# Kainmueller-Lab/PatchPerPix

Hardware: AMD Instinct MI355X
Metric: Mvoxels/sec assembled (vote_instances) (higher is better)
Workload: dtype f16 in, f32 accumulate

## Files before the change

include/ppp_mi355x.h:

```cpp
#ifndef PPP_MI355X_H
#define PPP_MI355X_H

#include <stddef.h>
#include <stdint.h>

#ifdef __cplusplus
extern "C" {
#endif

#define PPP_ABI_VERSION 5

enum ppp_error {
    PPP_OK = 0,
    PPP_ERR_INVALID_ARG = -1,
    PPP_ERR_NO_DEVICE = -2,
    PPP_ERR_HIP = -3,
    PPP_ERR_UNSUPPORTED = -4,
    PPP_ERR_WORKSPACE = -5
};

enum ppp_dtype { PPP_F32 = 0, PPP_F16 = 1, PPP_BF16 = 2 };

enum ppp_bg_rule { PPP_BG_INV_TH = 0, PPP_BG_HALF_TH = 1, PPP_BG_LESS_THAN_TH = 2 };
enum ppp_value_rule { PPP_VAL_COUNT = 0, PPP_VAL_PROB_PRODUCT = 1, PPP_VAL_NORM_PROB_PRODUCT = 2 };
// ... 44 lines not shown
int ppp_consensus_writes_voxel_major(const ppp_params *p);
int ppp_consensus_rows(const void *d_pred, int pred_dtype, const uint8_t *d_overlap, float *d_cons,
                       const ppp_params *p, void *stream);

int ppp_consensus_part(const void *d_pred, int pred_dtype, const uint8_t *d_overlap, float *d_cons,
                       const ppp_params *p, const ppp_box *part, void *stream);

int64_t ppp_consensus_sparse_workspace_bytes(const ppp_params *p, const ppp_box *part);
int ppp_consensus_sparse(const void *d_pred, int pred_dtype, const uint8_t *d_overlap, float *d_cons,
                         float *d_count, const ppp_params *p, const ppp_box *part, int open_rows, void *d_work,
                         int mode, void *stream);
void ppp_consensus_last_items(int64_t *total, int64_t *active, int *took_lists);

int ppp_rank_patches(const void *d_pred, int pred_dtype, const float *d_cons,
                     const uint8_t *d_overlap, float *d_score, const ppp_box *score_box,
                     const ppp_params *p, void *stream);

int64_t ppp_rank_workspace_bytes(const ppp_box *score_box, const ppp_params *p);
int ppp_rank_patches_vm(const void *d_pred, int pred_dtype, const float *d_cons_vm,
                        const uint8_t *d_overlap, float *d_score, const ppp_box *score_box,
                        void *d_work, const ppp_params *p, void *stream);
int ppp_rank_wg_plan(const ppp_box *score_box, const ppp_params *p, int resident_per_cu, int cus_per_xcd,
                     int32_t plan[8]);

int ppp_patch_graph(const void *d_pred, int pred_dtype, const float *d_cons,
                    const uint32_t *d_pairs, const uint32_t *d_order, uint64_t n_pairs,
                    float *d_aff, const ppp_params *p, void *stream);

int32_t ppp_patch_graph_by_patch_chunk(const ppp_params *p);
int32_t ppp_patch_graph_by_patch_chunk_small(const ppp_params *p);
int ppp_patch_graph_by_patch_chunked(const void *d_pred, int pred_dtype, const float *d_cons_vm,
                                     const uint32_t *d_pairs, const uint32_t *d_order,
                                     const int64_t *d_group_start, const int64_t *d_chunk_offsets,
                                     int32_t n_groups, int64_t n_blocks, int32_t chunk, float *d_aff,
                                     const ppp_params *p, void *stream);
int64_t ppp_patch_graph_lcg_words(int32_t dz, int32_t dy, int32_t dx, const ppp_params *p);
int ppp_patch_graph_lcg(const void *d_pred, int pred_dtype, const uint32_t *d_pairs,
                        const uint32_t *d_order, const int64_t *d_lcg_pos, int64_t n_lcg,
                        const int64_t *d_drop_off, uint64_t *d_drops, const ppp_params *p, void *stream);
int ppp_patch_graph_by_patch_lcg(const void *d_pred, int pred_dtype, const float *d_cons_vm,
                                 const uint32_t *d_pairs, const uint32_t *d_order,
                                 const int64_t *d_group_start, const int64_t *d_chunk_offsets,
                                 int32_t n_groups, int64_t n_blocks, int32_t chunk, float *d_aff,
                                 const int64_t *d_drop_off, const uint64_t *d_drops,
                                 const ppp_params *p, void *stream);
int ppp_patch_fg_bits(const void *d_pred, int pred_dtype, const int64_t *d_centres, int64_t n,
// ... 295 lines not shown
```

patchperpix_amd/backend.py:

```python
import ctypes
import os

import numpy as np

from . import build as _build

F32, F16, BF16 = 0, 1, 2
BG_INV_TH, BG_HALF_TH, BG_LESS_THAN_TH = 0, 1, 2
VAL_COUNT, VAL_PROB_PRODUCT, VAL_NORM_PROB_PRODUCT = 0, 1, 2
CONS_COMPACT, CONS_REFERENCE, CONS_VOXEL_MAJOR = 0, 1, 2
ABI_VERSION = 5
NONE_KEY = 0xFFFFFFFF
NONE_KEY64 = 1 << 62
PAIR_KEY_FAR = 0x7FFFFFFFFFFFFFFF


class Box(ctypes.Structure):
    _fields_ = [(n, ctypes.c_int32) for n in ("z0", "y0", "x0", "z1", "y1", "x1")]

    def shape(self):
        return (self.z1 - self.z0, self.y1 - self.y0, self.x1 - self.x0)


class Params(ctypes.Structure):
# ... 60 lines not shown
    "ppp_consensus": (ctypes.c_int, [ctypes.c_void_p, ctypes.c_int, ctypes.c_void_p,
                                     ctypes.c_void_p, ctypes.c_void_p,
                                     ctypes.POINTER(Params), ctypes.c_void_p]),
    "ppp_consensus_rows": (ctypes.c_int, [ctypes.c_void_p, ctypes.c_int, ctypes.c_void_p,
                                          ctypes.c_void_p, ctypes.POINTER(Params), ctypes.c_void_p]),
    "ppp_consensus_part": (ctypes.c_int, [ctypes.c_void_p, ctypes.c_int, ctypes.c_void_p,
                                          ctypes.c_void_p, ctypes.POINTER(Params), ctypes.POINTER(Box),
                                          ctypes.c_void_p]),
    "ppp_consensus_sparse_workspace_bytes": (ctypes.c_int64, [ctypes.POINTER(Params), ctypes.POINTER(Box)]),
    "ppp_consensus_sparse": (ctypes.c_int, [ctypes.c_void_p, ctypes.c_int, ctypes.c_void_p, ctypes.c_void_p,
                                            ctypes.c_void_p, ctypes.POINTER(Params), ctypes.POINTER(Box),
                                            ctypes.c_int, ctypes.c_void_p, ctypes.c_int, ctypes.c_void_p]),
    "ppp_consensus_last_items": (None, [ctypes.POINTER(ctypes.c_int64), ctypes.POINTER(ctypes.c_int64),
                                        ctypes.POINTER(ctypes.c_int)]),
    "ppp_cons_planes_to_rows": (ctypes.c_int, [ctypes.c_void_p, ctypes.POINTER(Box), ctypes.c_void_p,
                                               ctypes.POINTER(Params), ctypes.c_void_p]),
    "ppp_rank_patches": (ctypes.c_int, [ctypes.c_void_p, ctypes.c_int, ctypes.c_void_p,
                                        ctypes.c_void_p, ctypes.c_void_p,
                                        ctypes.POINTER(Box), ctypes.POINTER(Params),
                                        ctypes.c_void_p]),
    "ppp_rank_workspace_bytes": (ctypes.c_int64, [ctypes.POINTER(Box), ctypes.POINTER(Params)]),
    "ppp_rank_wg_plan": (ctypes.c_int, [ctypes.POINTER(Box), ctypes.POINTER(Params), ctypes.c_int, ctypes.c_int,
                                        ctypes.POINTER(ctypes.c_int32)]),
    "ppp_rank_patches_vm": (ctypes.c_int, [ctypes.c_void_p, ctypes.c_int, ctypes.c_void_p,
                                           ctypes.c_void_p, ctypes.c_void_p, ctypes.POINTER(Box),
                                           ctypes.c_void_p, ctypes.POINTER(Params), ctypes.c_void_p]),
    "ppp_patch_graph": (ctypes.c_int, [ctypes.c_void_p, ctypes.c_int, ctypes.c_void_p,
                                       ctypes.c_void_p, ctypes.c_void_p, ctypes.c_uint64,
                                       ctypes.c_void_p, ctypes.POINTER(Params),
                                       ctypes.c_void_p]),
    "ppp_patch_graph_by_patch": (ctypes.c_int, [ctypes.c_void_p, ctypes.c_int, ctypes.c_void_p,
                                                ctypes.c_void_p, ctypes.c_void_p, ctypes.c_void_p,
                                                ctypes.c_void_p, ctypes.c_int32, ctypes.c_int64,
                                                ctypes.c_void_p, ctypes.POINTER(Params),
                                                ctypes.c_void_p]),
    "ppp_patch_graph_by_patch_chunk_small": (ctypes.c_int32, [ctypes.POINTER(Params)]),
    "ppp_patch_graph_by_patch_chunked": (ctypes.c_int, [ctypes.c_void_p, ctypes.c_int, ctypes.c_void_p,
                                                        ctypes.c_void_p, ctypes.c_void_p, ctypes.c_void_p,
                                                        ctypes.c_void_p, ctypes.c_int32, ctypes.c_int64,
                                                        ctypes.c_int32, ctypes.c_void_p,
                                                        ctypes.POINTER(Params), ctypes.c_void_p]),
    "ppp_patch_graph_lcg_words": (ctypes.c_int64, [ctypes.c_int32, ctypes.c_int32, ctypes.c_int32,
                                                   ctypes.POINTER(Params)]),
    "ppp_patch_graph_lcg": (ctypes.c_int, [ctypes.c_void_p, ctypes.c_int, ctypes.c_void_p, ctypes.c_void_p,
                                           ctypes.c_void_p, ctypes.c_int64, ctypes.c_void_p, ctypes.c_void_p,
                                           ctypes.POINTER(Params), ctypes.c_void_p]),
# ... 689 lines not shown
        lo3 = [max(sb[a] - rad[a], (cb.z0, cb.y0, cb.x0)[a]) for a in range(3)]
        hi3 = [min(sb[3 + a] + rad[a], (cb.z1, cb.y1, cb.x1)[a]) for a in range(3)]
        note_add("s2_base_voxels", int(np.prod([max(0, h - l) for l, h in zip(lo3, hi3)])))
        with _timed("rank_patches"):
            check(lib().ppp_rank_patches_vm(_dev_ptr(pred), pred_dtype_code(pred), _dev_ptr(cons),
                                            _dev_ptr(overlap), _dev_ptr(out), box, _dev_ptr(work),
                                            ctypes.byref(P), _stream()))
        return out
    with _timed("rank_patches"):
        check(lib().ppp_rank_patches(_dev_ptr(pred), pred_dtype_code(pred), _dev_ptr(cons),
                                     _dev_ptr(overlap), _dev_ptr(out), box, ctypes.byref(P),
                                     _stream()))
    return out


def rank_wg_plan(P, score_box=None, resident_per_cu=0, cus_per_xcd=0):
    box = None if score_box is None else ctypes.byref(Box(*[int(v) for v in score_box]))
    out = (ctypes.c_int32 * 8)()
    check(lib().ppp_rank_wg_plan(box, ctypes.byref(P), int(resident_per_cu), int(cus_per_xcd), out))
    return dict(tile=(out[0], out[1], out[2]), tz_step=out[3], tiles=out[4], splits=out[5], slots=out[6],
                ranges="weight" if out[7] else "count")


def rank_vm_available(P):
    if os.environ.get("PPP_RANK", "vm") != "vm":
        return False
    Pv = P.copy()
    Pv.cons_layout = CONS_VOXEL_MAJOR
    Pv.cons_box = Box(0, 0, 0, P.Z, P.Y, P.X)
    if P.ring_z and P.ring_z < P.Z:
        Pv.cons_box = Box(0, 0, 0, P.ring_z, P.Y, P.X)
        sb = Box(0, 0, 0, max(1, P.ring_z - P.pz // 2), P.Y, P.X)
        return int(lib().ppp_rank_workspace_bytes(ctypes.byref(sb), ctypes.byref(Pv))) > 0
    return int(lib().ppp_rank_workspace_bytes(None, ctypes.byref(Pv))) > 0


def pair_order(pairs, P):
    torch = _torch()
    n = int(pairs.shape[0])
    keys = torch.empty((n,), dtype=torch.int64, device=pairs.device)
    check(lib().ppp_pair_sort_keys(_dev_ptr(pairs), n, _dev_ptr(keys), ctypes.byref(P), _stream()))
    return torch.argsort(keys).to(torch.int32)


def patch_graph_prepare(pred, pairs, Pv, ahead=False):
    import types
# ... 1249 lines not shown
```

patchperpix_amd/csrc/ppp_api.hip:

```cpp
#include <cmath>
#include <cstdarg>
#include <cstdio>
#include <cstring>

#include "ppp_kernels.hpp"

namespace {

thread_local char g_err[512] = "";

int fail(int code, const char *fmt, ...) {
    va_list ap;
    va_start(ap, fmt);
    vsnprintf(g_err, sizeof(g_err), fmt, ap);
    va_end(ap);
    return code;
}

int hip_fail(hipError_t e, const char *what) {
    return fail(PPP_ERR_HIP, "%s: %s", what, hipGetErrorString(e));
}

float round_down_f32(double t) {
    float f = (float)t;
// ... 288 lines not shown
int64_t ppp_rank_workspace_bytes(const ppp_box *score_box, const ppp_params *p) {
    ppp::Geo G;
    if (make_geo(p, &G) != PPP_OK) return -1;
    if (!ppp::rank_vm_supported(G)) return 0;
    if (G.ring && !ppp::rank_wg_supported(G)) return 0;
    ppp_box sb;
    if (rank_box(score_box, p, G, &sb) != PPP_OK) return -1;
    return (int64_t)ppp::rank_vm_workspace_bytes(sb, G);
}

int ppp_rank_wg_plan(const ppp_box *score_box, const ppp_params *p, int resident_per_cu, int cus_per_xcd, int32_t *plan) {
    ppp::Geo G;
    PPP_TRY(make_geo(p, &G));
    if (!plan) return fail(PPP_ERR_INVALID_ARG, "NULL pointer argument");
    if (!ppp::rank_wg_supported(G))
        return fail(PPP_ERR_UNSUPPORTED, "ppp_rank_wg_plan: the workgroup-per-tile kernel does not serve these parameters");
    ppp_box sb;
    PPP_TRY(rank_box(score_box, p, G, &sb));
    if (resident_per_cu <= 0 || cus_per_xcd <= 0) PPP_TRY(need_device());
    ppp::rank_wg_plan(sb, G, resident_per_cu, cus_per_xcd, plan);
    return PPP_OK;
}

#ifdef PPP_RW_STAMPS
extern "C" int64_t ppp_rank_wg_stamps_offset(const ppp_box *score_box, const ppp_params *p) {
    ppp::Geo G;
    ppp_box sb;
    if (make_geo(p, &G) != PPP_OK || !ppp::rank_wg_supported(G) || rank_box(score_box, p, G, &sb) != PPP_OK) return -1;
    return (int64_t)ppp::rank_wg_stamps_offset(sb, G);
}
#endif

int ppp_rank_patches_vm(const void *d_pred, int pred_dtype, const float *d_cons_vm,
                        const uint8_t *d_overlap, float *d_score, const ppp_box *score_box,
                        void *d_work, const ppp_params *p, void *stream) {
    ppp::Geo G;
    PPP_TRY(make_geo(p, &G));
    PPP_TRY(check_dtype(pred_dtype));
    if (!d_pred || !d_cons_vm || !d_score || !d_work) return fail(PPP_ERR_INVALID_ARG, "NULL pointer argument");
    if (G.use_overlap && !d_overlap) return fail(PPP_ERR_INVALID_ARG, "use_overlap set but d_overlap is NULL");
    if (!ppp::rank_vm_supported(G))
        return fail(PPP_ERR_UNSUPPORTED, "ppp_rank_patches_vm: VOXEL_MAJOR layout, cubic patches of 3/5/7/9, "
                                         "no count_pos_neg (use ppp_rank_patches otherwise)");
    if (G.ring && !ppp::rank_wg_supported(G))
        return fail(PPP_ERR_UNSUPPORTED, "ring_z: only the workgroup-per-tile ranking kernel reads a ring of rows");
    ppp_box sb;
// ... 1314 lines not shown
```

patchperpix_amd/csrc/ppp_kernels.hpp:

```cpp
#pragma once
#include <stdlib.h>
#include <string.h>
#include "ppp_common.hpp"

namespace ppp {

int env_epoch();
void env_reload();
struct EnvSwitch {
    const char *name;
    int seen = -1;
    bool is_set = false;
    char val[32] = {0};
    explicit EnvSwitch(const char *n) : name(n) {}
    const char *get() {
        if (seen != env_epoch()) {
            const char *e = getenv(name);
            is_set = e != nullptr;
            if (e) { strncpy(val, e, sizeof(val) - 1); val[sizeof(val) - 1] = 0; }
            seen = env_epoch();
        }
        return is_set ? val : nullptr;
    }
};
// ... 17 lines not shown
                                const Geo &G, void *work, int mode, long long *total, long long *active,
                                int *took_lists, hipStream_t s);
void note_consensus_kernel(const char *name);
int last_consensus_short_form();
void note_consensus_short_form(int on);
const char *last_rank_kernel();
void note_rank_kernel(const char *name);
const char *last_patch_graph_kernel();
const char *last_patch_graph_geometry();
void note_patch_graph_kernel(const char *name, const char *geometry = "none");
hipError_t launch_consensus_part(const void *pred, int dtype, const uint8_t *ov, float *cons, const Geo &G,
                                 hipStream_t s);
hipError_t launch_rank(const void *pred, int dtype, const float *cons, const uint8_t *ov,
                       float *score, const ppp_box &sb, const Geo &G, hipStream_t s);
hipError_t launch_rank_v2(const void *pred, int dtype, const float *cons, const uint8_t *ov,
                          float *score, const ppp_box &sb, const Geo &G, hipStream_t s);
bool rank_vm_supported(const Geo &G);
size_t rank_vm_workspace_bytes(const ppp_box &sb, const Geo &G);
hipError_t launch_rank_vm(const void *pred, int dtype, const float *S, const uint8_t *ov, float *score,
                          const ppp_box &sb, void *work, const Geo &G, hipStream_t s);
bool rank_wg_supported(const Geo &G);
size_t rank_wg_workspace_bytes(const ppp_box &sb, const Geo &G);
void rank_wg_plan(const ppp_box &sb, const Geo &G, int resident_per_cu, int cus_per_xcd, int32_t out[8]);
#ifdef PPP_RW_STAMPS
size_t rank_wg_stamps_offset(const ppp_box &sb, const Geo &G);
#endif
hipError_t launch_rank_wg(const void *pred, int dtype, const float *S, const uint8_t *ov, float *score,
                          const ppp_box &sb, void *work, const Geo &G, hipStream_t s);
hipError_t launch_patch_graph(const void *pred, int dtype, const float *cons,
                              const uint32_t *pairs, const uint32_t *order, uint64_t n,
                              float *aff, const Geo &G, hipStream_t s);
int patch_graph_pa_chunk(const Geo &G, bool small = false);
hipError_t launch_patch_graph_pa(const void *pred, int dtype, const float *S, const uint32_t *rows,
                                 const uint32_t *order, const long long *group_start,
                                 const long long *chunk_offsets, int n_groups, long long n_blocks,
                                 int chunk, float *aff, const long long *drop_off,
                                 const unsigned long long *drops, const long long *bits_centres, int n_bits,
                                 const uint32_t *bits, const Geo &G, hipStream_t s);
hipError_t launch_patch_fg_bits(const void *pred, int dtype, const long long *centres, long long n,
                                uint32_t *table, const Geo &G, hipStream_t s);
long long patch_graph_lcg_words(const Geo &G, int dz, int dy, int dx);
hipError_t launch_patch_graph_lcg(const void *pred, int dtype, const uint32_t *rows, const uint32_t *order,
                                  const long long *lcg_pos, long long n, const long long *drop_off,
                                  unsigned long long *drops, const Geo &G, hipStream_t s);
hipError_t launch_label(const uint32_t *pairs, const float *aff, uint64_t n,
                        const uint32_t *nodes, uint64_t n_nodes, uint32_t *node_key, void *work,
// ... 175 lines not shown
```

patchperpix_amd/csrc/ppp_rank_wg.hip:

```cpp
#include <stdlib.h>
#include <string.h>

#include <type_traits>

#include "ppp_kernels.hpp"

namespace ppp {

static constexpr int RW_MINWAVES = 4;
static constexpr bool rw_zruns(int PX) { return PX == 9; }
static constexpr bool rw_bankdeal(int PX) { return PX == 7; }
static constexpr int RW_PAD = 8;
static constexpr int RW_WAVES = 4;
static constexpr int rw_mask_words(int C) { return (((C + 15) / 16) + 3) & ~3; }
__host__ __device__ __forceinline__ long long rw_mask_quad0(long long zy, int x, int sX, int quads) {
    return ((zy * ((sX + 15) >> 4) + (x >> 4)) * quads) * 16 + (x & 15);
}
static constexpr int RW_QSTRIDE = 16;
static size_t rw_mask_bytes(int sZ, int sY, int sX, int C) {
    const size_t cols = (size_t)((sX + 15) >> 4) * 16;
    return (size_t)sZ * sY * cols * rw_mask_words(C) * 4;
}
typedef const volatile __attribute__((address_space(3))) float *lds_f32_cvp2;

typedef _Float16 rw_h2 __attribute__((ext_vector_type(2)));
__device__ __forceinline__ float fma_mix_lo(float r, uint32_t c, float acc) {
    return __builtin_fmaf(r, (float)__builtin_bit_cast(rw_h2, c).x, acc);
}
__device__ __forceinline__ float fma_mix_hi(float r, uint32_t c, float acc) {
    return __builtin_fmaf(r, (float)__builtin_bit_cast(rw_h2, c).y, acc);
}

template <int I, int END>
struct StaticFor {
    template <class F>
    static __device__ __forceinline__ void run(F &&f) {
// ... 211 lines not shown
    for (int az = 0; az < nz; ++az)
        for (int ay = 0; ay < ny; ++ay) {
            const int ax = (r - SY * ay - SZ * az) & 31;
            if (ax >= nx) continue;
            const uint16_t e = (uint16_t)(0x8000 | (az << 8) | (ay << 4) | ax);
            if (k < H) slot[32 * k + r] = e;
            else if (k - H < MAXOVER) over[r][k - H] = e;
            ++k;
        }
    n_over[r] = k > H ? min(k - H, MAXOVER) : 0;
    __syncthreads();
    if (r == 0) {
        int f = 0;
        for (int rr = 0; rr < 32; ++rr)
            for (int o = 0; o < n_over[rr]; ++o) {
                while (f < 32 * H && slot[f] != 0) ++f;
                if (f < 32 * H) slot[f] = over[rr][o];
            }
    }
    __syncthreads();
    for (int i = r; i < SLOTS; i += 32) T[(size_t)cls * SLOTS + i] = slot[i];
}

template <int PZ, int PY, int PX, int TZ, int TY, int TX, bool DZ = false>
__global__ void __launch_bounds__(64 * RW_WAVES, RW_MINWAVES)
    rank_wg_kernel(const float *__restrict__ S, const uint32_t *__restrict__ M,
                   const uint32_t *__restrict__ info, const uint8_t *__restrict__ valid,
                   float *__restrict__ score, const ppp_box sb, const Geo G, const int tiles_y,
                   const int tiles_x, const int n_tiles, const int32_t *__restrict__ order, const int y_major, const uint16_t *__restrict__ dealT,
                   const int tz_step
#ifdef PPP_RW_STAMPS
                   , uint32_t *__restrict__ stamps
#endif
                   ) {
#ifdef PPP_RW_STAMPS
    const unsigned long long t_start = wall_clock64();
#endif
    constexpr int C = PZ * PY * PX, W16 = (C + 15) / 16, RZ = PZ / 2, RY = PY / 2, RX = PX / 2;
    constexpr int W16P = rw_mask_words(C);
    constexpr int NMW = W16;
    constexpr int WZ = 2 * PZ - 1, WY = 2 * PY - 1, WX = 2 * PX - 1, W = WZ * WY * WX, LC = (W - 1) / 2;
    constexpr int NTHR = 64 * RW_WAVES;
    constexpr int NST = (W + NTHR - 1) / NTHR;
    constexpr int NT = TZ * TY * TX;
    constexpr int UB = (TZ + 2 * RZ) * (TY + 2 * RY) * (TX + 2 * RX);
    constexpr int SZ = WY * WX;
    constexpr int SZP = rw_zruns(PX) ? SZ + ((9 - SZ % 32) + 32) % 32 : SZ;
    constexpr int LCP = LC + (PZ - 1) * (SZP - SZ);
    auto img = [](int e) -> int { return SZP == SZ ? e : (e / SZ) * SZP + e % SZ; };
    __shared__ float rowbuf[WZ * SZP + 2 * RW_PAD];
    __shared__ float accs[NT];
    __shared__ uint32_t act_bits[(NT + 31) / 32];
    __shared__ uint2 coefT[256];
    __shared__ uint32_t uvalid_bits[(UB + 63) / 64 * 2];
    __shared__ int any_act;
    const int tid = threadIdx.x, lane = tid & 63;
    const int wave = __builtin_amdgcn_readfirstlane(tid >> 6);
    const int sX = sb.x1 - sb.x0, sY = sb.y1 - sb.y0, sZ = sb.z1 - sb.z0;
    const long long sbV = (long long)sX * sY * sZ;
    const int n_blocks = gridDim.x;
    const int per_xcd = (n_blocks + 7) / 8;
    const int slot = (blockIdx.x & 7) * per_xcd + (blockIdx.x >> 3);
    const int rec = order ? order[slot] : slot;
    if (rec < 0) return;
    const int bid = rec & RW_TILE_MASK, half_hi = (rec & RW_HALF_HI) ? 1 : 0, halved = (rec & (RW_HALF_LO | RW_HALF_HI)) ? 1 : 0;
    if (bid >= n_tiles) return;
    int tx_i, ty_i, tz_i;
    rw_tile_decode(bid, n_tiles, tiles_y, tiles_x, y_major, tz_i, ty_i, tx_i);
    const int tzs = DZ ? min(tz_step, TZ) : TZ;
    const int c0z = sb.z0 + tz_i * tzs, c0y = sb.y0 + ty_i * TY + half_hi * (TY / 2), c0x = sb.x0 + tx_i * TX;
    const int tz = min(tzs, sb.z1 - c0z), ty = min(halved ? TY / 2 : TY, sb.y1 - c0y), tx = min(TX, sb.x1 - c0x);
    if (tz <= 0 || ty <= 0 || tx <= 0) return;

    auto sb_index = [&](int lz, int ly, int lx) -> long long {
        return ((long long)(c0z + lz - sb.z0) * sY + (c0y + ly - sb.y0)) * sX + (c0x + lx - sb.x0);
    };
    for (int e = tid; e < 256; e += NTHR) {
// ... 96 lines not shown
        const int uk_next = __builtin_amdgcn_readfirstlane(next_valid(uk + 1));
        if (uk_next < nu) {
            const float *src = row_src(uk_next);
#pragma unroll
            for (int i = 0; i < NST; ++i) {
                const int e = tid + i * NTHR;
                st[i] = e < W ? src[e] : 0.0f;
            }
        }
        const RowG R = row_geom(uk);
        const int n_box = R.n_box;
        const int first = (wave + RW_WAVES - turn) % RW_WAVES;
        turn = (turn + ((n_box + 63) >> 6)) % RW_WAVES;
        for (int i0 = 64 * first; i0 < n_box; i0 += NTHR) {
            const ItemG it = item_geom(R, i0);
            const int ax = it.ax, ay = it.ay, az = it.az, cl = it.cl, a = it.a;
            const long long q0 = it.q0;
            bool active = it.in && ((act_bits[cl >> 5] >> (cl & 31)) & 1u) != 0;
            uint32_t mw[NMW];
            if (active)
                active = ((M[(q0 + (long long)(a >> 6) * RW_QSTRIDE) * 4 + ((a >> 4) & 3)] >> (8 * ((a >> 2) & 3) + (a & 3))) & 1u) != 0;
            if (__ballot(active) == 0) continue;
            const uint4 *mc = reinterpret_cast<const uint4 *>(M) + q0;
#pragma unroll
            for (int q = 0; q < W16P / 4; ++q) {
                const uint4 v = mc[q * RW_QSTRIDE];
                if (4 * q < NMW) mw[4 * q] = v.x;
                if (4 * q + 1 < NMW) mw[4 * q + 1] = v.y;
                if (4 * q + 2 < NMW) mw[4 * q + 2] = v.z;
                if (4 * q + 3 < NMW) mw[4 * q + 3] = v.w;
            }
#pragma unroll
            for (int w = 0; w < W16; ++w) mw[w] = active ? mw[w] : 0u;
            float acc = active ? accs[cl] : 0.0f;
            lds_f32_cvp2 row = (lds_f32_cvp2)(rowbuf + RW_PAD + LCP - (az * SZP + ay * WX + ax));
            lds_f32_cvp2 rowc[4];
#pragma unroll
            for (int i2 = 0; i2 < 4; ++i2) rowc[i2] = row;
            const int aw = a >> 4;
            const uint32_t above16 = ~((2u << (a & 15)) - 1u) & 0xFFFFu;
            const uint32_t keep_a = interleave16(above16, 0xFFFFu);
            StaticFor<0, W16>::run([&](auto wc) {
                constexpr int w = decltype(wc)::value;
                const uint32_t m = mw[w] & (w < aw ? 0xF0F0F0F0u : (w > aw ? 0xFFFFFFFFu : keep_a));
                if (__ballot(m != 0u) == 0) return;
                uint2 cf[4];
#pragma unroll
                for (int j = 0; j < 4; ++j)
                    if (w * 16 + j * 4 < C) cf[j] = coefT[(m >> (8 * j)) & 0xFFu];
                float rv[2][4];
                auto load_rows = [&](int j, float (&r)[4]) {
#pragma unroll
                    for (int i3 = 0; i3 < 4; ++i3) {
                        const int i2 = 3 - i3;
                        const int b = w * 16 + j * 4 + i2;
                        if (b < C) r[i2] = rowc[i2][(b / (PY * PX)) * SZP + ((b / PX) % PY) * WX + b % PX];
                    }
                };
                load_rows(0, rv[0]);
                if (w * 16 + 4 < C) load_rows(1, rv[1]);
#pragma unroll
                for (int j = 0; j < 4; ++j) {
                    if (w * 16 + j * 4 < C) {
                        float r0[4];
#pragma unroll
                        for (int i2 = 0; i2 < 4; ++i2) r0[i2] = rv[j & 1][i2];
// ... 64 lines not shown
    RankWgWork W;
    W.M = (uint32_t *)c.take_bytes(rw_mask_bytes(sZ, sY, sX, G.C));
    W.info = c.take<uint32_t>((size_t)sX * sY * sZ);
    W.valid = c.take<uint8_t>(G.V);
    W.weight = c.take<int32_t>(RW_ORDER_MAX);
    W.order = c.take<int32_t>(RW_ORDER_MAX);
    W.dealT = (uint16_t *)c.take_bytes(rw_deal_bytes(G.px));
    return W;
}
size_t rank_wg_workspace_bytes(const ppp_box &sb, const Geo &G) { Carver c(nullptr); rank_wg_layout(c, sb, G); return c.used; }
#ifdef PPP_RW_STAMPS
size_t rank_wg_stamps_offset(const ppp_box &sb, const Geo &G) {
    char base;
    Carver c(&base);
    return (size_t)((char *)rank_wg_layout(c, sb, G).weight - &base);
}
#endif

static int rw_choose_splits(int tiles_per_xcd, int slots_per_xcd) {
    if (slots_per_xcd <= 0 || tiles_per_xcd <= slots_per_xcd) return 0;
    const int rem = tiles_per_xcd % slots_per_xcd;
    return 2 * rem <= slots_per_xcd ? rem : 0;
}
template <int P, bool FIT>
static int rw_resident_per_cu() {
    static thread_local int memo = 0;
    if (memo == 0) {
        int nb = 0;
        hipError_t e;
        if constexpr (FIT) e = hipOccupancyMaxActiveBlocksPerMultiprocessor(&nb, rank_wg_kernel<P, P, P, 16, 16, 16, true>, 64 * RW_WAVES, 0);
        else e = hipOccupancyMaxActiveBlocksPerMultiprocessor(&nb, rank_wg_kernel<P, P, P, 8, 16, 16>, 64 * RW_WAVES, 0);
        if (e != hipSuccess || nb < 1) nb = RW_MINWAVES;
        memo = nb;
    }
    return memo;
}
static int rw_cus_per_xcd() {
    static thread_local int memo = 0;
    if (memo == 0) {
        int dev = 0, cus = 0;
        if (hipGetDevice(&dev) != hipSuccess || hipDeviceGetAttribute(&cus, hipDeviceAttributeMultiprocessorCount, dev) != hipSuccess || cus < 8)
            cus = 256;
        memo = cus / 8;
    }
    return memo;
}

struct RwPlan {
    int TZ, TY, TX;
    int tz_step;
    bool fit;
    int tiles_z, tiles_y, tiles_x;
    long long n_tiles;
    int per_xcd, splits, slots;
    bool ordered, by_weight;
};
static int rw_env_int(EnvSwitch &sw, int none) {
    const char *e = sw.get();
    return (e && e[0] >= '0' && e[0] <= '9') ? atoi(e) : none;
}
static RwPlan rw_plan(const ppp_box &sb, const Geo &G, int resident, int resident_fit, int cus_per_xcd) {
    const int sX = sb.x1 - sb.x0, sY = sb.y1 - sb.y0, sZ = sb.z1 - sb.z0;
    RwPlan p{};
    const long long big_tiles = (long long)((sZ + 7) / 8) * ((sY + 15) / 16) * ((sX + 15) / 16);
    bool big = big_tiles >= 4 * 256;
    static EnvSwitch tile_sw("PPP_RANK_WG_TILE");
    if (const char *e = tile_sw.get()) big = strcmp(e, "8x16x16") == 0 ? true : (strcmp(e, "8x8x16") == 0 ? false : big);
    if (rw_zruns(G.px) && !tile_sw.get()) big = false;
    bool tall = tile_sw.get() && strcmp(tile_sw.get(), "16x8x16") == 0;
    if (G.rank_tile && !tile_sw.get()) { big = G.rank_tile == 2; tall = G.rank_tile == 3; }
    const bool by_rule = big && !tall && !tile_sw.get() && !G.rank_tile;
    p.TZ = tall ? 16 : 8; p.TY = tall ? 8 : (big ? 16 : 8); p.TX = 16;
    p.tz_step = p.TZ;
    static EnvSwitch order_sw("PPP_RANK_ORDER");
    static EnvSwitch split_sw("PPP_RANK_WG_SPLIT");
    static EnvSwitch tz_sw("PPP_RANK_WG_TZ");
    static EnvSwitch xcd_sw("PPP_RANK_WG_XCD");
    const int split_env = rw_env_int(split_sw, -1);
    const int tz_env = G.px == 7 ? rw_env_int(tz_sw, 0) : 0;
    const int slots_res = resident * cus_per_xcd, slots_fit = resident_fit * cus_per_xcd;
    auto tiles_of = [&](int t, int ty) { return (long long)((sZ + t - 1) / t) * ((sY + ty - 1) / ty) * ((sX + 15) / 16); };
    if (tz_env > 0) {
        p.fit = true; p.TZ = 16; p.TY = 16; p.TX = 16;
        p.tz_step = tz_env < 16 ? tz_env : 16;
    } else if (by_rule && G.px == 7 && split_env < 0) {
        const long long per0 = (tiles_of(8, 16) + 7) / 8;
        if (slots_res > 0 && per0 > slots_res && per0 < 2LL * slots_res)
            for (int t = 9; t <= 16; ++t)
                if ((tiles_of(t, 16) + 7) / 8 <= slots_fit) { p.fit = true; p.TZ = 16; p.tz_step = t; break; }
    }
    p.tiles_z = (sZ + p.tz_step - 1) / p.tz_step; p.tiles_y = (sY + p.TY - 1) / p.TY; p.tiles_x = (sX + p.TX - 1) / p.TX;
    p.n_tiles = (long long)p.tiles_z * p.tiles_y * p.tiles_x;
    p.per_xcd = (int)((p.n_tiles + 7) / 8);
    p.ordered = !(p.n_tiles > RW_ORDER_MAX || (order_sw.get() && order_sw.get()[0] == '0'));
    p.slots = p.per_xcd;
    if (p.ordered) {
        if (split_env >= 0) p.splits = split_env;
        else if (by_rule && !p.fit) p.splits = rw_choose_splits(p.per_xcd, slots_res);
        p.splits = p.splits < p.per_xcd ? p.splits : p.per_xcd;
        if (8LL * (p.per_xcd + p.splits) > RW_ORDER_MAX) p.splits = RW_ORDER_MAX / 8 - p.per_xcd;
        p.by_weight = p.fit && tz_env == 0;
        if (const char *e = xcd_sw.get()) p.by_weight = strcmp(e, "weight") == 0 ? true : (strcmp(e, "count") == 0 ? false : p.by_weight);
        p.slots = p.per_xcd + p.splits;
        if (p.by_weight) {
            p.slots += (p.per_xcd + 3) / 4;
            if (8LL * p.slots > RW_ORDER_MAX) p.slots = RW_ORDER_MAX / 8;
        }
    }
    return p;
}
static RwPlan rw_plan_device(const ppp_box &sb, const Geo &G) {
    const int res = G.px == 5 ? rw_resident_per_cu<5, false>() : (G.px == 7 ? rw_resident_per_cu<7, false>() : rw_resident_per_cu<9, false>());
    return rw_plan(sb, G, res, G.px == 7 ? rw_resident_per_cu<7, true>() : res, rw_cus_per_xcd());
}
void rank_wg_plan(const ppp_box &sb, const Geo &G, int resident_per_cu, int cus_per_xcd, int32_t out[8]) {
    const RwPlan p = (resident_per_cu > 0 && cus_per_xcd > 0) ? rw_plan(sb, G, resident_per_cu, resident_per_cu, cus_per_xcd)
                                                              : rw_plan_device(sb, G);
    out[0] = p.TZ; out[1] = p.TY; out[2] = p.TX; out[3] = p.tz_step;
    out[4] = (int32_t)p.n_tiles; out[5] = p.splits; out[6] = p.slots; out[7] = p.by_weight ? 1 : 0;
}

template <typename T>
static hipError_t launch_rwg(const T *pred, const float *S, const uint8_t *ov, float *score,
                             const ppp_box &sb, void *work, const Geo &G, hipStream_t s) {
    const int sX = sb.x1 - sb.x0, sY = sb.y1 - sb.y0, sZ = sb.z1 - sb.z0;
    const size_t sbV = (size_t)sX * sY * sZ;
    Carver carver(work);
    auto [M, info, valid, weight, order, dealT] = rank_wg_layout(carver, sb, G);
    if (!cons_box_covers(G, sb)) return hipErrorInvalidValue;
    PPP_GRID_CHECK((G.V + 255) / 256, 256);
    PPP_GRID_CHECK((sbV + 255) / 256, 256);
    rank_valid2_kernel<T><<<dim3((unsigned)((G.V + 255) / 256)), dim3(256), 0, s>>>(pred, ov, valid, G);
    note_rank_kernel("rank_wg_kernel");
    const dim3 pre_grid((unsigned)((sbV + 255) / 256));
#define PPP_RW_PRE(P)                                                                                       \
    case P:                                                                                                 \
        rank_masks_il_kernel<T, P><<<pre_grid, dim3(256), 0, s>>>(pred, valid, sb, M, info, score, G);      \
        break;
    switch (G.px) {
        PPP_RW_PRE(5)
        PPP_RW_PRE(7)
        PPP_RW_PRE(9)
// ... 3 lines not shown
    const RwPlan plan = rw_plan_device(sb, G);
    const bool tall = plan.TZ == 16 && !plan.fit, big = plan.TY == 16, fit = plan.fit;
    const int tiles_y = plan.tiles_y, tiles_x = plan.tiles_x, per_xcd = plan.per_xcd, splits = plan.splits, tz_step = plan.tz_step;
    const long long n_tiles = plan.n_tiles;
    if (!plan.ordered) order = nullptr;
    const long long n_blocks = 8LL * plan.slots;
    PPP_GRID_CHECK(n_blocks, 64 * RW_WAVES);
    static EnvSwitch major_sw("PPP_RANK_TILE_MAJOR");
    const int y_major = (major_sw.get() && major_sw.get()[0] == 'z') ? 0 : 1;
    if (order) {
        rank_tile_weight_kernel<<<dim3((unsigned)n_tiles), dim3(256), 0, s>>>(info, valid, sb, tz_step, plan.TY, plan.TX, tiles_y, tiles_x,
                                                                              y_major, weight, G);
        rank_tile_order_kernel<<<dim3(8), dim3(256), 0, s>>>(weight, (int)n_tiles, per_xcd, splits, plan.slots,
                                                             plan.by_weight ? 1 : 0, order);
    }
    if (rw_bankdeal(G.px))
        rank_deal_table_kernel<7><<<dim3(7 * 7 * 7), dim3(32), 0, s>>>(dealT, 2 * 7 - 1, (2 * 7 - 1) * (2 * 7 - 1));
#ifdef PPP_RW_STAMPS
    (void)hipMemsetAsync(weight, 0, (size_t)RW_ORDER_MAX * 4, s);
#define PPP_RW_STAMP_ARG , (uint32_t *)weight
#else
#define PPP_RW_STAMP_ARG
#endif
#define PPP_RW_LAUNCH(A_, D_, E_, F_, DZ_)                                                                  \
    rank_wg_kernel<A_, A_, A_, D_, E_, F_, DZ_><<<dim3((unsigned)n_blocks), dim3(64 * RW_WAVES), 0, s>>>(   \
        S, M, info, valid, score, sb, G, tiles_y, tiles_x, (int)n_tiles, order, y_major, dealT, tz_step PPP_RW_STAMP_ARG)
#define PPP_RW_CASE(P)                                                                                      \
    case P:                                                                                                 \
        if (tall) PPP_RW_LAUNCH(P, 16, 8, 16, false);                                                       \
        else if (big) PPP_RW_LAUNCH(P, 8, 16, 16, false);                                                   \
        else PPP_RW_LAUNCH(P, 8, 8, 16, false);                                                             \
        break;
    if (fit) {
        if (G.px != 7) return hipErrorNotSupported;
        PPP_RW_LAUNCH(7, 16, 16, 16, true);
    } else
    switch (G.px) {
        PPP_RW_CASE(5)
        PPP_RW_CASE(7)
        PPP_RW_CASE(9)
    default:
        return hipErrorNotSupported;
    }
#undef PPP_RW_LAUNCH
#undef PPP_RW_STAMP_ARG
#undef PPP_RW_CASE
#undef PPP_RW_PRE
    return hipGetLastError();
}

hipError_t launch_rank_wg(const void *pred, int dtype, const float *S, const uint8_t *ov, float *score,
                          const ppp_box &sb, void *work, const Geo &G, hipStream_t s) {
    if (!rank_wg_supported(G)) return hipErrorNotSupported;
    return with_pred_type(dtype, [&](auto tag) {
        using T = PPP_PRED_T(tag);
        return launch_rwg<T>((const T *)pred, S, ov, score, sb, work, G, s);
    });
}

}
```

Measured before the change: 16.40.

## Size fit-path rank kernel LDS to z-step and raise its occupancy target

The fit path of the rank workgroup kernel now instantiates variants with tile depth 8/10/12/16 matched to the chosen z-step, so LDS use shrinks with smaller steps. These variants are compiled with a higher minimum-waves launch bound and load mask quads lazily inside the word loop to cut register pressure. The planner queries occupancy per variant and may pick the fit path even at z-step 8. This aims at more resident workgroups per CU and fewer tail slots, at the cost of more template instantiations and possible register spills.

```diff
diff --git a/include/ppp_mi355x.h b/include/ppp_mi355x.h
--- a/include/ppp_mi355x.h
+++ b/include/ppp_mi355x.h
@@ -90,6 +90,8 @@
                         void *d_work, const ppp_params *p, void *stream);
 int ppp_rank_wg_plan(const ppp_box *score_box, const ppp_params *p, int resident_per_cu, int cus_per_xcd,
                      int32_t plan[8]);
+int ppp_rank_wg_plan_residency(const ppp_box *score_box, const ppp_params *p, int resident_per_cu, int cus_per_xcd,
+                               int32_t res[4]);
 
 int ppp_patch_graph(const void *d_pred, int pred_dtype, const float *d_cons,
                     const uint32_t *d_pairs, const uint32_t *d_order, uint64_t n_pairs,
diff --git a/patchperpix_amd/backend.py b/patchperpix_amd/backend.py
--- a/patchperpix_amd/backend.py
+++ b/patchperpix_amd/backend.py
@@ -106,6 +106,8 @@
     "ppp_rank_workspace_bytes": (ctypes.c_int64, [ctypes.POINTER(Box), ctypes.POINTER(Params)]),
     "ppp_rank_wg_plan": (ctypes.c_int, [ctypes.POINTER(Box), ctypes.POINTER(Params), ctypes.c_int, ctypes.c_int,
                                         ctypes.POINTER(ctypes.c_int32)]),
+    "ppp_rank_wg_plan_residency": (ctypes.c_int, [ctypes.POINTER(Box), ctypes.POINTER(Params), ctypes.c_int,
+                                                  ctypes.c_int, ctypes.POINTER(ctypes.c_int32)]),
     "ppp_rank_patches_vm": (ctypes.c_int, [ctypes.c_void_p, ctypes.c_int, ctypes.c_void_p,
                                            ctypes.c_void_p, ctypes.c_void_p, ctypes.POINTER(Box),
                                            ctypes.c_void_p, ctypes.POINTER(Params), ctypes.c_void_p]),
@@ -841,6 +843,13 @@
                 ranges="weight" if out[7] else "count")
 
 
+def rank_wg_plan_residency(P, score_box=None, resident_per_cu=0, cus_per_xcd=0):
+    box = None if score_box is None else ctypes.byref(Box(*[int(v) for v in score_box]))
+    out = (ctypes.c_int32 * 4)()
+    check(lib().ppp_rank_wg_plan_residency(box, ctypes.byref(P), int(resident_per_cu), int(cus_per_xcd), out))
+    return dict(lds_tz=out[0], resident=out[1], lds_bytes=out[2], cus_per_xcd=out[3])
+
+
 def rank_vm_available(P):
     if os.environ.get("PPP_RANK", "vm") != "vm":
         return False
diff --git a/patchperpix_amd/csrc/ppp_api.hip b/patchperpix_amd/csrc/ppp_api.hip
--- a/patchperpix_amd/csrc/ppp_api.hip
+++ b/patchperpix_amd/csrc/ppp_api.hip
@@ -334,6 +334,19 @@
     return PPP_OK;
 }
 
+int ppp_rank_wg_plan_residency(const ppp_box *score_box, const ppp_params *p, int resident_per_cu, int cus_per_xcd, int32_t *res) {
+    ppp::Geo G;
+    PPP_TRY(make_geo(p, &G));
+    if (!res) return fail(PPP_ERR_INVALID_ARG, "NULL pointer argument");
+    if (!ppp::rank_wg_supported(G))
+        return fail(PPP_ERR_UNSUPPORTED, "ppp_rank_wg_plan_residency: the workgroup-per-tile kernel does not serve these parameters");
+    ppp_box sb;
+    PPP_TRY(rank_box(score_box, p, G, &sb));
+    if (resident_per_cu <= 0 || cus_per_xcd <= 0) PPP_TRY(need_device());
+    ppp::rank_wg_plan_residency(sb, G, resident_per_cu, cus_per_xcd, res);
+    return PPP_OK;
+}
+
 #ifdef PPP_RW_STAMPS
 extern "C" int64_t ppp_rank_wg_stamps_offset(const ppp_box *score_box, const ppp_params *p) {
     ppp::Geo G;
diff --git a/patchperpix_amd/csrc/ppp_kernels.hpp b/patchperpix_amd/csrc/ppp_kernels.hpp
--- a/patchperpix_amd/csrc/ppp_kernels.hpp
+++ b/patchperpix_amd/csrc/ppp_kernels.hpp
@@ -63,6 +63,7 @@
 bool rank_wg_supported(const Geo &G);
 size_t rank_wg_workspace_bytes(const ppp_box &sb, const Geo &G);
 void rank_wg_plan(const ppp_box &sb, const Geo &G, int resident_per_cu, int cus_per_xcd, int32_t out[8]);
+void rank_wg_plan_residency(const ppp_box &sb, const Geo &G, int resident_per_cu, int cus_per_xcd, int32_t out[4]);
 #ifdef PPP_RW_STAMPS
 size_t rank_wg_stamps_offset(const ppp_box &sb, const Geo &G);
 #endif
diff --git a/patchperpix_amd/csrc/ppp_rank_wg.hip b/patchperpix_amd/csrc/ppp_rank_wg.hip
--- a/patchperpix_amd/csrc/ppp_rank_wg.hip
+++ b/patchperpix_amd/csrc/ppp_rank_wg.hip
@@ -12,6 +12,10 @@
 static constexpr bool rw_bankdeal(int PX) { return PX == 7; }
 static constexpr int RW_PAD = 8;
 static constexpr int RW_WAVES = 4;
+static constexpr int RW_FIT_MINWAVES = 6;
+static constexpr int RW_FIT_NTZ = 4;
+static constexpr int RW_FIT_TZ[RW_FIT_NTZ] = {8, 10, 12, 16};
+static constexpr int rw_fit_index(int tz_step) { return tz_step <= 8 ? 0 : (tz_step <= 10 ? 1 : (tz_step <= 12 ? 2 : 3)); }
 static constexpr int rw_mask_words(int C) { return (((C + 15) / 16) + 3) & ~3; }
 __host__ __device__ __forceinline__ long long rw_mask_quad0(long long zy, int x, int sX, int quads) {
     return ((zy * ((sX + 15) >> 4) + (x >> 4)) * quads) * 16 + (x & 15);
@@ -269,8 +273,22 @@
     for (int i = r; i < SLOTS; i += 32) T[(size_t)cls * SLOTS + i] = slot[i];
 }
 
-template <int PZ, int PY, int PX, int TZ, int TY, int TX, bool DZ = false>
-__global__ void __launch_bounds__(64 * RW_WAVES, RW_MINWAVES)
+template <int P, int TZ, int TY, int TX>
+struct RwLds {
+    static constexpr int W1 = 2 * P - 1, SZ = W1 * W1;
+    static constexpr int SZP = rw_zruns(P) ? SZ + ((9 - SZ % 32) + 32) % 32 : SZ;
+    static constexpr int ROW = W1 * SZP + 2 * RW_PAD;
+    static constexpr int NT = TZ * TY * TX;
+    static constexpr int ACT = (NT + 31) / 32;
+    static constexpr int UB = (TZ + 2 * (P / 2)) * (TY + 2 * (P / 2)) * (TX + 2 * (P / 2));
+    static constexpr int UV = (UB + 63) / 64 * 2;
+    static constexpr int up16(int b) { return (b + 15) & ~15; }
+    static constexpr int bytes = up16(4 * ROW) + up16(4 * NT) + up16(4 * ACT) + 256 * 8 + up16(4 * UV) + 16;
+};
+static constexpr int RW_LDS_PER_CU = 160 * 1024;
+
+template <int PZ, int PY, int PX, int TZ, int TY, int TX, bool DZ = false, int MINW = RW_MINWAVES>
+__global__ void __launch_bounds__(64 * RW_WAVES, MINW)
     rank_wg_kernel(const float *__restrict__ S, const uint32_t *__restrict__ M,
                    const uint32_t *__restrict__ info, const uint8_t *__restrict__ valid,
                    float *__restrict__ score, const ppp_box sb, const Geo G, const int tiles_y,
@@ -295,11 +313,13 @@
     constexpr int SZP = rw_zruns(PX) ? SZ + ((9 - SZ % 32) + 32) % 32 : SZ;
     constexpr int LCP = LC + (PZ - 1) * (SZP - SZ);
     auto img = [](int e) -> int { return SZP == SZ ? e : (e / SZ) * SZP + e % SZ; };
-    __shared__ float rowbuf[WZ * SZP + 2 * RW_PAD];
-    __shared__ float accs[NT];
-    __shared__ uint32_t act_bits[(NT + 31) / 32];
+    using Lds = RwLds<PX, TZ, TY, TX>;
+    static_assert(PZ == PX && PY == PX && Lds::ROW == WZ * SZP + 2 * RW_PAD && Lds::NT == NT && Lds::UB == UB, "RwLds restates these arrays");
+    __shared__ float rowbuf[Lds::ROW];
+    __shared__ float accs[Lds::NT];
+    __shared__ uint32_t act_bits[Lds::ACT];
     __shared__ uint2 coefT[256];
-    __shared__ uint32_t uvalid_bits[(UB + 63) / 64 * 2];
+    __shared__ uint32_t uvalid_bits[Lds::UV];
     __shared__ int any_act;
     const int tid = threadIdx.x, lane = tid & 63;
     const int wave = __builtin_amdgcn_readfirstlane(tid >> 6);
@@ -442,6 +462,18 @@
                 active = ((M[(q0 + (long long)(a >> 6) * RW_QSTRIDE) * 4 + ((a >> 4) & 3)] >> (8 * ((a >> 2) & 3) + (a & 3))) & 1u) != 0;
             if (__ballot(active) == 0) continue;
             const uint4 *mc = reinterpret_cast<const uint4 *>(M) + q0;
+            constexpr bool LAZY = DZ && MINW > RW_MINWAVES;
+            auto load_quad = [&](auto qc) {
+                constexpr int q = decltype(qc)::value;
+                const uint4 v = mc[q * RW_QSTRIDE];
+                if (4 * q < NMW) mw[4 * q] = active ? v.x : 0u;
+                if (4 * q + 1 < NMW) mw[4 * q + 1] = active ? v.y : 0u;
+                if (4 * q + 2 < NMW) mw[4 * q + 2] = active ? v.z : 0u;
+                if (4 * q + 3 < NMW) mw[4 * q + 3] = active ? v.w : 0u;
+            };
+            if constexpr (LAZY) {
+                load_quad(std::integral_constant<int, 0>{});
+            } else {
 #pragma unroll
             for (int q = 0; q < W16P / 4; ++q) {
                 const uint4 v = mc[q * RW_QSTRIDE];
@@ -452,6 +484,7 @@
             }
 #pragma unroll
             for (int w = 0; w < W16; ++w) mw[w] = active ? mw[w] : 0u;
+            }
             float acc = active ? accs[cl] : 0.0f;
             lds_f32_cvp2 row = (lds_f32_cvp2)(rowbuf + RW_PAD + LCP - (az * SZP + ay * WX + ax));
             lds_f32_cvp2 rowc[4];
@@ -462,6 +495,7 @@
             const uint32_t keep_a = interleave16(above16, 0xFFFFu);
             StaticFor<0, W16>::run([&](auto wc) {
                 constexpr int w = decltype(wc)::value;
+                if constexpr (LAZY && w % 4 == 0 && w / 4 + 1 < W16P / 4) load_quad(std::integral_constant<int, w / 4 + 1>{});
                 const uint32_t m = mw[w] & (w < aw ? 0xF0F0F0F0u : (w > aw ? 0xFFFFFFFFu : keep_a));
                 if (__ballot(m != 0u) == 0) return;
                 uint2 cf[4];
@@ -572,18 +606,24 @@
     const int rem = tiles_per_xcd % slots_per_xcd;
     return 2 * rem <= slots_per_xcd ? rem : 0;
 }
-template <int P, bool FIT>
+template <int P, bool FIT, int TZ = 8>
 static int rw_resident_per_cu() {
     static thread_local int memo = 0;
     if (memo == 0) {
         int nb = 0;
         hipError_t e;
-        if constexpr (FIT) e = hipOccupancyMaxActiveBlocksPerMultiprocessor(&nb, rank_wg_kernel<P, P, P, 16, 16, 16, true>, 64 * RW_WAVES, 0);
+        if constexpr (FIT) e = hipOccupancyMaxActiveBlocksPerMultiprocessor(&nb, rank_wg_kernel<P, P, P, TZ, 16, 16, true, RW_FIT_MINWAVES>, 64 * RW_WAVES, 0);
         else e = hipOccupancyMaxActiveBlocksPerMultiprocessor(&nb, rank_wg_kernel<P, P, P, 8, 16, 16>, 64 * RW_WAVES, 0);
         if (e != hipSuccess || nb < 1) nb = RW_MINWAVES;
         memo = nb;
     }
     return memo;
+}
+static int rw_lds_bytes(int P, bool fit, int TZ, int TY) {
+    if (fit) return TZ <= 8 ? RwLds<7, 8, 16, 16>::bytes : (TZ <= 10 ? RwLds<7, 10, 16, 16>::bytes : (TZ <= 12 ? RwLds<7, 12, 16, 16>::bytes : RwLds<7, 16, 16, 16>::bytes));
+#define PPP_RW_LDS(P_) (TZ == 16 ? RwLds<P_, 16, 8, 16>::bytes : (TY == 16 ? RwLds<P_, 8, 16, 16>::bytes : RwLds<P_, 8, 8, 16>::bytes))
+    return P == 5 ? PPP_RW_LDS(5) : (P == 7 ? PPP_RW_LDS(7) : PPP_RW_LDS(9));
+#undef PPP_RW_LDS
 }
 static int rw_cus_per_xcd() {
     static thread_local int memo = 0;
@@ -600,6 +640,8 @@
     int TZ, TY, TX;
     int tz_step;
     bool fit;
+    int lds_tz;
+    int resident, lds_bytes;
     int tiles_z, tiles_y, tiles_x;
     long long n_tiles;
     int per_xcd, splits, slots;
@@ -609,7 +651,9 @@
     const char *e = sw.get();
     return (e && e[0] >= '0' && e[0] <= '9') ? atoi(e) : none;
 }
-static RwPlan rw_plan(const ppp_box &sb, const Geo &G, int resident, int resident_fit, int cus_per_xcd) {
+struct RwResident { int base, fit[RW_FIT_NTZ]; };
+static RwPlan rw_plan(const ppp_box &sb, const Geo &G, const RwResident &res, int cus_per_xcd) {
+    const int resident = res.base;
     const int sX = sb.x1 - sb.x0, sY = sb.y1 - sb.y0, sZ = sb.z1 - sb.z0;
     RwPlan p{};
     const long long big_tiles = (long long)((sZ + 7) / 8) * ((sY + 15) / 16) * ((sX + 15) / 16);
@@ -628,7 +672,7 @@
     static EnvSwitch xcd_sw("PPP_RANK_WG_XCD");
     const int split_env = rw_env_int(split_sw, -1);
     const int tz_env = G.px == 7 ? rw_env_int(tz_sw, 0) : 0;
-    const int slots_res = resident * cus_per_xcd, slots_fit = resident_fit * cus_per_xcd;
+    const int slots_res = resident * cus_per_xcd;
     auto tiles_of = [&](int t, int ty) { return (long long)((sZ + t - 1) / t) * ((sY + ty - 1) / ty) * ((sX + 15) / 16); };
     if (tz_env > 0) {
         p.fit = true; p.TZ = 16; p.TY = 16; p.TX = 16;
@@ -636,9 +680,12 @@
     } else if (by_rule && G.px == 7 && split_env < 0) {
         const long long per0 = (tiles_of(8, 16) + 7) / 8;
         if (slots_res > 0 && per0 > slots_res && per0 < 2LL * slots_res)
-            for (int t = 9; t <= 16; ++t)
-                if ((tiles_of(t, 16) + 7) / 8 <= slots_fit) { p.fit = true; p.TZ = 16; p.tz_step = t; break; }
-    }
+            for (int t = 8; t <= 16; ++t)
+                if ((tiles_of(t, 16) + 7) / 8 <= (long long)res.fit[rw_fit_index(t)] * cus_per_xcd) { p.fit = true; p.TZ = 16; p.tz_step = t; break; }
+    }
+    p.lds_tz = p.fit ? RW_FIT_TZ[rw_fit_index(p.tz_step)] : p.TZ;
+    p.resident = p.fit ? res.fit[rw_fit_index(p.tz_step)] : resident;
+    p.lds_bytes = rw_lds_bytes(G.px, p.fit, p.lds_tz, p.TY);
     p.tiles_z = (sZ + p.tz_step - 1) / p.tz_step; p.tiles_y = (sY + p.TY - 1) / p.TY; p.tiles_x = (sX + p.TX - 1) / p.TX;
     p.n_tiles = (long long)p.tiles_z * p.tiles_y * p.tiles_x;
     p.per_xcd = (int)((p.n_tiles + 7) / 8);
@@ -660,14 +707,36 @@
     return p;
 }
 static RwPlan rw_plan_device(const ppp_box &sb, const Geo &G) {
-    const int res = G.px == 5 ? rw_resident_per_cu<5, false>() : (G.px == 7 ? rw_resident_per_cu<7, false>() : rw_resident_per_cu<9, false>());
-    return rw_plan(sb, G, res, G.px == 7 ? rw_resident_per_cu<7, true>() : res, rw_cus_per_xcd());
+    RwResident res;
+    res.base = G.px == 5 ? rw_resident_per_cu<5, false>() : (G.px == 7 ? rw_resident_per_cu<7, false>() : rw_resident_per_cu<9, false>());
+    for (int i = 0; i < RW_FIT_NTZ; ++i) res.fit[i] = res.base;
+    if (G.px == 7) {
+        res.fit[0] = rw_resident_per_cu<7, true, 8>(); res.fit[1] = rw_resident_per_cu<7, true, 10>();
+        res.fit[2] = rw_resident_per_cu<7, true, 12>(); res.fit[3] = rw_resident_per_cu<7, true, 16>();
+    }
+    return rw_plan(sb, G, res, rw_cus_per_xcd());
+}
+static RwPlan rw_plan_assumed(const ppp_box &sb, const Geo &G, int resident, int cus_per_xcd) {
+    RwResident res;
+    res.base = resident;
+    for (int i = 0; i < RW_FIT_NTZ; ++i) {
+        const int by_lds = RW_LDS_PER_CU / rw_lds_bytes(7, true, RW_FIT_TZ[i], 16);
+        res.fit[i] = resident < by_lds ? resident : by_lds;
+    }
+    return rw_plan(sb, G, res, cus_per_xcd);
 }
 void rank_wg_plan(const ppp_box &sb, const Geo &G, int resident_per_cu, int cus_per_xcd, int32_t out[8]) {
-    const RwPlan p = (resident_per_cu > 0 && cus_per_xcd > 0) ? rw_plan(sb, G, resident_per_cu, resident_per_cu, cus_per_xcd)
+    const RwPlan p = (resident_per_cu > 0 && cus_per_xcd > 0) ? rw_plan_assumed(sb, G, resident_per_cu, cus_per_xcd)
                                                               : rw_plan_device(sb, G);
     out[0] = p.TZ; out[1] = p.TY; out[2] = p.TX; out[3] = p.tz_step;
     out[4] = (int32_t)p.n_tiles; out[5] = p.splits; out[6] = p.slots; out[7] = p.by_weight ? 1 : 0;
+}
+void rank_wg_plan_residency(const ppp_box &sb, const Geo &G, int resident_per_cu, int cus_per_xcd, int32_t out[4]) {
+    const bool assumed = resident_per_cu > 0 && cus_per_xcd > 0;
+    const RwPlan p = assumed ? rw_plan_assumed(sb, G, resident_per_cu, cus_per_xcd) : rw_plan_device(sb, G);
+    const int by_lds = RW_LDS_PER_CU / p.lds_bytes;
+    out[0] = p.lds_tz; out[1] = (assumed && by_lds < p.resident) ? by_lds : p.resident; out[2] = p.lds_bytes;
+    out[3] = assumed ? cus_per_xcd : rw_cus_per_xcd();
 }
 
 template <typename T>
@@ -717,9 +786,12 @@
 #else
 #define PPP_RW_STAMP_ARG
 #endif
+#define PPP_RW_ARGS S, M, info, valid, score, sb, G, tiles_y, tiles_x, (int)n_tiles, order, y_major, dealT, tz_step PPP_RW_STAMP_ARG
 #define PPP_RW_LAUNCH(A_, D_, E_, F_, DZ_)                                                                  \
-    rank_wg_kernel<A_, A_, A_, D_, E_, F_, DZ_><<<dim3((unsigned)n_blocks), dim3(64 * RW_WAVES), 0, s>>>(   \
-        S, M, info, valid, score, sb, G, tiles_y, tiles_x, (int)n_tiles, order, y_major, dealT, tz_step PPP_RW_STAMP_ARG)
+    rank_wg_kernel<A_, A_, A_, D_, E_, F_, DZ_><<<dim3((unsigned)n_blocks), dim3(64 * RW_WAVES), 0, s>>>(PPP_RW_ARGS)
+#define PPP_RW_LAUNCH_FIT(TZ_)                                                                              \
+    rank_wg_kernel<7, 7, 7, TZ_, 16, 16, true, RW_FIT_MINWAVES>                                             \
+        <<<dim3((unsigned)n_blocks), dim3(64 * RW_WAVES), 0, s>>>(PPP_RW_ARGS)
 #define PPP_RW_CASE(P)                                                                                      \
     case P:                                                                                                 \
         if (tall) PPP_RW_LAUNCH(P, 16, 8, 16, false);                                                       \
@@ -728,7 +800,12 @@
         break;
     if (fit) {
         if (G.px != 7) return hipErrorNotSupported;
-        PPP_RW_LAUNCH(7, 16, 16, 16, true);
+        switch (plan.lds_tz) {
+        case 8: PPP_RW_LAUNCH_FIT(8); break;
+        case 10: PPP_RW_LAUNCH_FIT(10); break;
+        case 12: PPP_RW_LAUNCH_FIT(12); break;
+        default: PPP_RW_LAUNCH_FIT(16); break;
+        }
     } else
     switch (G.px) {
         PPP_RW_CASE(5)
@@ -738,6 +815,8 @@
         return hipErrorNotSupported;
     }
 #undef PPP_RW_LAUNCH
+#undef PPP_RW_LAUNCH_FIT
+#undef PPP_RW_ARGS
 #undef PPP_RW_STAMP_ARG
 #undef PPP_RW_CASE
 #undef PPP_RW_PRE
```

New measurement: 16.77, median of 6. +2.3%, better.
